# gargatik/Seamless-Through-Breaking-Rethinking-Image-Stitching-for-Optimal-Alignment

Measured on AMD Instinct MI355X. Metric: stitched image-pairs/s at 512x512, higher is better.
Workload: dtype f32 (decoder contractions, PatchEmbed's third conv and the C = 128 block tails: exact 3xbf16 split of both operands, 6 products on the bf16 matrix cores, fp32 accumulate -- error vs fp64 0.83x the fp32 MFMA chain's; everything else fp32); 1 GPU; UDIS-D-shaped 512x512 pairs, batch=1, FlowHomoAdpater.forward(type=test_eval); launch=hipGraph replay, pairs_in_flight=3

## Files before the change

### include/stitch_gfx950.h

```cpp
#ifndef STITCH_GFX950_H
#define STITCH_GFX950_H
#include <stdint.h>
#ifdef __cplusplus
extern "C" {
#endif

typedef struct st_gemm_desc {
    const float* a;
    const float* w;
    float* c;
    const float* bias;
    const float* aux0;
    const float* aux1;
    const float* aux2;
    const float* scale_ptr;
    int32_t M, N, K;
    int32_t H, W, Cin, ldx;
    int32_t kh, kw, sh, sw, ph, pw, Ho, Wo;
    int32_t ldw, ldc, ld_aux0, ld_aux1, ld_aux2;
    int32_t aux0_row_div, aux0_row_mod;
    int32_t act;
    int32_t epi;
    float alpha;
    int32_t batch;
// ... 124 lines not shown
int st_copy2d(const float* src, int32_t lds, float* dst, int32_t ldd, int32_t rows, int32_t cols, void* stream);
int st_prep_image(const float* src, float* dst, int32_t B, int32_t C, int32_t H, int32_t W, int32_t ldo,
                  float mul, float div, float sub, void* stream);

int st_latent_pool(const float* scores, int32_t ld_s, const float* tokens, int32_t ld_t, float* z, int32_t pixels,
                   int32_t P, void* stream);

int st_coords_grid(float* out, int32_t B, int32_t H, int32_t W, void* stream);
int st_coords_grid_init(float* out, const float* init, int32_t B, int32_t H, int32_t W, void* stream);
int st_flow_forward_interpolate(const float* src, int32_t src_is_coords_rows, float* out, int32_t B, int32_t H, int32_t W,
                                void* stream);
int st_flow_from_coords(const float* coords1, float* flow4, int32_t ld4, float* dst2, int32_t ld2, int32_t B,
                        int32_t H, int32_t W, void* stream);
int st_flow_encode(const float* coords1, const float* w98, const float* bias, float* out, int32_t ldo, float* flow2,
                   int32_t ld2, int32_t B, int32_t H, int32_t W, int32_t Co, void* stream);
int st_flow_encode_split3(const float* coords1, const float* w98, const float* bias, float* out, int32_t ldo, float* flow2,
                          int32_t ld2, int32_t B, int32_t H, int32_t W, int32_t Co, void* out_planes, int64_t out_pstride,
                          int64_t out_prows, void* flow_planes, int64_t flow_pstride, int64_t flow_prows, int32_t flow_col,
                          void* stream);
int st_cost_lookup(const float* maps, const float* coords, float* out, int32_t ldo, int32_t Nq, int32_t H2,
                   int32_t W2, int32_t r, void* stream);
int st_decoder_token_chain(float* corr, int32_t ld_corr, const float* coords1, const float* kv,
                           const float* const* weights16, int32_t rows, int32_t ntok, void* stream);
int st_convex_upsample(const float* coords1, const float* mask, int32_t ldm, float* out, int32_t B, int32_t H,
                       int32_t W, void* stream);

int st_dlt4(const float* src4x2, const float* motion, float* H, int32_t B, float mscale_x, float mscale_y,
            float div, void* stream);
int st_mat3_sandwich(const float* L, const float* X, const float* R, float* out, int32_t B, int32_t invert,
                     void* stream);
int st_homo_warp(const float* U, const float* theta, float* out, int32_t* idx, int32_t B, int32_t C,
                 int32_t n_ones, int32_t H, int32_t W, int32_t oh, int32_t ow, void* stream);
int st_mesh_bounds(const float* H, float* out4, int32_t B, float width, float height, int32_t gw, int32_t gh,
                   void* stream);
int st_flow_warp(const float* x, const float* flow, const float* mul, float* out, int32_t B, int32_t C,
                 int32_t H, int32_t W, void* stream);
int st_homo_flow_warp(const float* image2, const float* H8, const float* flow, float* out6, float* overlap, float* Hi,
                      int32_t B, int32_t H, int32_t W, void* stream);
int st_resize_bilinear(const float* x, float* out, int32_t planes, int32_t H, int32_t W, int32_t oh, int32_t ow,
                       int32_t align_corners, float div0, float div1, int32_t ndiv, void* stream);
int st_range_map(const float* flow, void* scratch_u64, float* out, int32_t B, int32_t H, int32_t W, void* stream);
int st_occlusion_from_range(const float* range, float* out, int64_t n, int32_t threshold, void* stream);
int st_morph_open(const float* mask, float* out, void* scratch_u8x2, int32_t N, int32_t H, int32_t W,
                  int32_t ksz, void* stream);
int st_eval_finish(float* final6, const float* occ, float* overlap, int32_t B, int32_t H, int32_t W, void* stream);
int st_blend(const float* homo1, const float* homo2, float* fin, const float* occ, float* output2, float* mask1,
// ... 169 lines not shown
```

### seamless-through-breaking-rethinking-image-stitching-for-optimal-alignment_amd/csrc/flowops.hip

```cpp
#include "common.h"
#include <type_traits>
#include "../../include/stitch_gfx950.h"

__global__ void coords_grid_kernel(float* __restrict__ out, int B, int H, int W) {
    const size_t idx = (size_t)blockIdx.x * blockDim.x + threadIdx.x;
    if (idx >= (size_t)B * H * W) return;
    const int r = idx % ((size_t)H * W);
    out[idx * 2] = (float)(r % W);
    out[idx * 2 + 1] = (float)(r / W);
}

extern "C" int st_coords_grid(float* out, int32_t B, int32_t H, int32_t W, void* stream) {
    if (!out || B <= 0 || H <= 0 || W <= 0) return ST_EINVAL;
    const size_t total = (size_t)B * H * W;
    hipLaunchKernelGGL(coords_grid_kernel, dim3((total + 255) / 256), dim3(256), 0, (hipStream_t)stream, out, B, H, W);
    ST_CHECK_LAUNCH();
    return ST_OK;
}

__global__ void coords_grid_init_kernel(float* __restrict__ out, const float* __restrict__ init, int B, int H, int W) {
    const size_t idx = (size_t)blockIdx.x * blockDim.x + threadIdx.x;
    if (idx >= (size_t)B * H * W) return;
    const size_t N = (size_t)H * W, b = idx / N;
    const int r = idx % N;
// ... 13 lines not shown
                                        float* __restrict__ dst2, int ld2, int B, int H, int W) {
    const size_t idx = (size_t)blockIdx.x * blockDim.x + threadIdx.x;
    if (idx >= (size_t)B * H * W) return;
    const int r = idx % ((size_t)H * W);
    const float fx = coords1[idx * 2] - (float)(r % W);
    const float fy = coords1[idx * 2 + 1] - (float)(r / W);
    if (flow4) {
        flow4[idx * ld4] = fx; flow4[idx * ld4 + 1] = fy;
        for (int c = 2; c < ld4; ++c) flow4[idx * ld4 + c] = 0.f;
    }
    if (dst2) { dst2[idx * ld2] = fx; dst2[idx * ld2 + 1] = fy; }
}

extern "C" int st_flow_from_coords(const float* coords1, float* flow4, int32_t ld4, float* dst2, int32_t ld2, int32_t B,
                                   int32_t H, int32_t W, void* stream) {
    if (!coords1 || B <= 0 || H <= 0 || W <= 0 || (flow4 && ld4 < 2) || (dst2 && ld2 < 2)) return ST_EINVAL;
    const size_t total = (size_t)B * H * W;
    hipLaunchKernelGGL(flow_from_coords_kernel, dim3((total + 255) / 256), dim3(256), 0, (hipStream_t)stream, coords1, flow4,
                       ld4, dst2, ld2, B, H, W);
    ST_CHECK_LAUNCH();
    return ST_OK;
}

__global__ __launch_bounds__(512) void flow_encode_kernel(const float* __restrict__ coords1, const float* __restrict__ w,
                                                          const float* __restrict__ bias, float* __restrict__ out, int ldo,
                                                          float* __restrict__ flow2, int ld2, int H, int W, int Co,
                                                          __bf16* __restrict__ out_planes, long long out_pstride, long long out_prows,
                                                          __bf16* __restrict__ flow_planes, long long flow_pstride, long long flow_prows, int flow_col) {
    __shared__ float2 patch[10 * 14];
    __shared__ __attribute__((aligned(16))) float wsm[98 * 128];
    const int tid = threadIdx.x, lane = tid & 63, wave = __builtin_amdgcn_readfirstlane(tid >> 6);
    const int tiles_x = (W + 7) >> 3;
    const int b = blockIdx.z, ty = (int)blockIdx.x / tiles_x, tx = (int)blockIdx.x - ty * tiles_x;
    const size_t img = (size_t)b * H * W;
    const int cbase = (int)blockIdx.y * 128;
    {
        float4 v[7];
#pragma unroll
        for (int u = 0; u < 7; ++u) {
            const int f = u * 512 + tid, t = f >> 5, c4 = (f & 31) * 4;
            v[u] = make_float4(0.f, 0.f, 0.f, 0.f);
            if (t < 98 && cbase + c4 < Co) v[u] = *reinterpret_cast<const float4*>(w + (size_t)t * Co + cbase + c4);
        }
#pragma unroll
        for (int u = 0; u < 7; ++u) {
            const int f = u * 512 + tid;
            if (f < 98 * 32) *reinterpret_cast<float4*>(wsm + f * 4) = v[u];
        }
    }
    if (tid < 140) {
        const int py = tid / 14, px = tid - py * 14;
        const int y = ty * 4 + py - 3, x = tx * 8 + px - 3;
        float2 f = make_float2(0.f, 0.f);
        if (y >= 0 && y < H && x >= 0 && x < W) {
            const float2 cc = *reinterpret_cast<const float2*>(coords1 + (img + (size_t)y * W + x) * 2);
            f = make_float2(cc.x - (float)x, cc.y - (float)y);
        }
        patch[tid] = f;
// ... 25 lines not shown
                acc[p] = fmaf(f[p + kx].y, wr[kx * 2 + 1], acc[p]);
            }
    }
#pragma unroll
    for (int p = 0; p < 8; ++p) {
        const int x = tx * 8 + p;
        if (x < W && cok) {
            const float o = fmaxf(acc[p], 0.f);
            out[(img + (size_t)y * W + x) * ldo + c] = o;
            if (out_planes) {
                __bf16 h, m, l;
                st_split3(o, h, m, l);
                const unsigned ph = st_bf16_bits(h), pm = st_bf16_bits(m), pl = st_bf16_bits(l);
                const unsigned nh = (unsigned)__builtin_amdgcn_update_dpp(0, (int)ph, 0xB1, 0xF, 0xF, false);
                const unsigned nm = (unsigned)__builtin_amdgcn_update_dpp(0, (int)pm, 0xB1, 0xF, 0xF, false);
                const unsigned nl = (unsigned)__builtin_amdgcn_update_dpp(0, (int)pl, 0xB1, 0xF, 0xF, false);
                if (!(c & 1)) {
                    unsigned* pp = reinterpret_cast<unsigned*>(out_planes + ((size_t)(c >> 5) * out_prows + img + (size_t)y * W + x) * 32 + (c & 31));
                    pp[0] = ph | (nh << 16); pp[out_pstride / 2] = pm | (nm << 16); pp[out_pstride] = pl | (nl << 16);
                }
            }
        }
    }
    if (flow2 && blockIdx.y == 0 && (wave & 1) == 0 && lane < 8 && tx * 8 + lane < W) {
        const float2 f = patch[(row + 3) * 14 + lane + 3];
        const size_t r = img + (size_t)y * W + tx * 8 + lane;
        flow2[r * ld2] = f.x; flow2[r * ld2 + 1] = f.y;
        if (flow_planes) {
            __bf16 hx, mx, lx, hy, my, ly;
            unsigned* pp = reinterpret_cast<unsigned*>(flow_planes + ((size_t)(flow_col >> 5) * flow_prows + r) * 32 + (flow_col & 31));
            st_split3(f.x, hx, mx, lx);
            st_split3(f.y, hy, my, ly);
            pp[0] = st_bf16_bits(hx) | ((unsigned)st_bf16_bits(hy) << 16);
            pp[flow_pstride / 2] = st_bf16_bits(mx) | ((unsigned)st_bf16_bits(my) << 16);
            pp[flow_pstride] = st_bf16_bits(lx) | ((unsigned)st_bf16_bits(ly) << 16);
        }
    }
}

extern "C" int st_flow_encode(const float* coords1, const float* w98, const float* bias, float* out, int32_t ldo, float* flow2,
                              int32_t ld2, int32_t B, int32_t H, int32_t W, int32_t Co, void* stream) {
    if (!coords1 || !w98 || !bias || !out || B <= 0 || H <= 0 || W <= 0 || Co <= 0 || (Co & 3) || ((uintptr_t)w98 & 15)) return ST_EINVAL;
    if (ldo < Co || (flow2 && ld2 < 2) || ((uintptr_t)coords1 & 7)) return ST_EINVAL;
    dim3 grid(((H + 3) / 4) * ((W + 7) / 8), (Co + 127) / 128, B);
    hipLaunchKernelGGL(flow_encode_kernel, grid, dim3(512), 0, (hipStream_t)stream, coords1, w98, bias, out, ldo, flow2, ld2, H, W, Co,
                       (__bf16*)nullptr, 0LL, 0LL, (__bf16*)nullptr, 0LL, 0LL, 0);
    ST_CHECK_LAUNCH();
    return ST_OK;
}

extern "C" int st_flow_encode_split3(const float* coords1, const float* w98, const float* bias, float* out, int32_t ldo, float* flow2,
                                     int32_t ld2, int32_t B, int32_t H, int32_t W, int32_t Co, void* out_planes, int64_t out_pstride,
                                     int64_t out_prows, void* flow_planes, int64_t flow_pstride, int64_t flow_prows, int32_t flow_col,
                                     void* stream) {
    if (!coords1 || !w98 || !bias || !out || B <= 0 || H <= 0 || W <= 0 || Co <= 0 || (Co & 31) || ((uintptr_t)w98 & 15)) return ST_EINVAL;
    if (ldo < Co || (flow2 && ld2 < 2) || ((uintptr_t)coords1 & 7)) return ST_EINVAL;
    if (!out_planes || out_pstride <= 0 || out_prows < (int64_t)B * H * W) return ST_EINVAL;
    if (flow_planes && (!flow2 || flow_pstride <= 0 || flow_prows < (int64_t)B * H * W || flow_col < 0 || (flow_col & 1))) return ST_EINVAL;
    dim3 grid(((H + 3) / 4) * ((W + 7) / 8), (Co + 127) / 128, B);
    hipLaunchKernelGGL(flow_encode_kernel, grid, dim3(512), 0, (hipStream_t)stream, coords1, w98, bias, out, ldo, flow2, ld2, H, W, Co,
                       (__bf16*)out_planes, (long long)out_pstride, (long long)out_prows, (__bf16*)flow_planes, (long long)flow_pstride,
                       (long long)flow_prows, (int)flow_col);
    ST_CHECK_LAUNCH();
    return ST_OK;
}

__global__ __launch_bounds__(256) void cost_lookup_kernel(const float* __restrict__ maps, const float* __restrict__ coords,
                                                          float* __restrict__ out, int ldo, int Nq, int H2, int W2, int r) {
#pragma clang fp contract(off)
    const int side = 2 * r + 1, nch = side * side;
    const size_t idx = (size_t)blockIdx.x * 256 + threadIdx.x;
    if (idx >= (size_t)Nq * nch) return;
    const int ch = idx % nch;
    const size_t n = idx / nch;
    const int i = ch / side, j = ch % side;
    const float x = coords[n * 2] + (float)(i - r);
    const float y = coords[n * 2 + 1] + (float)(j - r);
    const float gx = 2.0f * x / (float)(W2 - 1) - 1.0f, gy = 2.0f * y / (float)(H2 - 1) - 1.0f;
    const float ix = ((gx + 1.0f) / 2.0f) * (float)(W2 - 1), iy = ((gy + 1.0f) / 2.0f) * (float)(H2 - 1);
    const float x0f = floorf(ix), y0f = floorf(iy);
    const int x0 = (int)x0f, y0 = (int)y0f, x1 = x0 + 1, y1 = y0 + 1;
    const float x1f = x0f + 1.0f, y1f = y0f + 1.0f;
    const float nw = (x1f - ix) * (y1f - iy), ne = (ix - x0f) * (y1f - iy);
    const float sw = (x1f - ix) * (iy - y0f), se = (ix - x0f) * (iy - y0f);
    const float* m = maps + n * (size_t)(H2 * W2);
    const bool xin0 = x0 >= 0 && x0 < W2, xin1 = x1 >= 0 && x1 < W2;
    const bool yin0 = y0 >= 0 && y0 < H2, yin1 = y1 >= 0 && y1 < H2;
    float v = (xin0 && yin0 ? m[y0 * W2 + x0] : 0.f) * nw;
    v = __fmaf_rn(xin1 && yin0 ? m[y0 * W2 + x1] : 0.f, ne, v);
    v = __fmaf_rn(xin0 && yin1 ? m[y1 * W2 + x0] : 0.f, sw, v);
    v = __fmaf_rn(xin1 && yin1 ? m[y1 * W2 + x1] : 0.f, se, v);
    out[n * ldo + ch] = v;
}

extern "C" int st_cost_lookup(const float* maps, const float* coords, float* out, int32_t ldo, int32_t Nq, int32_t H2,
                              int32_t W2, int32_t r, void* stream) {
    if (!maps || !coords || !out || Nq <= 0 || r < 0 || r > 64 || ldo < (2 * r + 1) * (2 * r + 1)) return ST_EINVAL;
    if (H2 < 2 || W2 < 2 || (int64_t)H2 * W2 > 0x7fffffff) return ST_EINVAL;
    const size_t total = (size_t)Nq * (2 * r + 1) * (2 * r + 1);
    hipLaunchKernelGGL(cost_lookup_kernel, dim3((total + 255) / 256), dim3(256), 0, (hipStream_t)stream, maps, coords, out,
                       ldo, Nq, H2, W2, r);
    ST_CHECK_LAUNCH();
    return ST_OK;
}

__global__ __launch_bounds__(256) void convex_upsample_kernel(const float* __restrict__ coords1, const float* __restrict__ mask,
                                                              int ldm, float* __restrict__ out, int B, int H, int W) {
    const size_t gid = (size_t)blockIdx.x * 256 + threadIdx.x;
    const size_t pix = gid >> 6;
    if (pix >= (size_t)B * H * W) return;
    const int sub = gid & 63, i = sub >> 3, j = sub & 7;
    const int b = pix / ((size_t)H * W), r = pix % ((size_t)H * W);
    const int y = r / W, x = r % W;
    const float* mp = mask + pix * ldm + sub;
    float mv[9], mx = -INFINITY;
// ... 82 lines not shown
    for (int r = 0; r < 4; ++r) {
        mh[r] = sum16(v[0][r] + v[1][r]) * (1.0f / 32.0f);
        const float d0 = v[0][r] - mh[r], d1 = v[1][r] - mh[r];
        m2h[r] = sum16(d0 * d0 + d1 * d1);
        if (c == 0) { red_mine[(4 * g + r) * 2] = mh[r]; red_mine[(4 * g + r) * 2 + 1] = m2h[r]; }
    }
    __syncthreads();
#pragma unroll
    for (int r = 0; r < 4; ++r) {
        const float mo = red_other[(4 * g + r) * 2], m2o = red_other[(4 * g + r) * 2 + 1];
        const float mean = 0.5f * (mh[r] + mo), d = mh[r] - mo;
        const float var = ((m2h[r] + m2o) + d * d * 16.0f) * (1.0f / 64.0f);
        const float rstd = 1.0f / sqrtf(var + 1e-5f);
#pragma unroll
        for (int t = 0; t < 2; ++t) v[t][r] = (v[t][r] - mean) * rstd * w[col0 + 16 * t + c] + b[col0 + 16 * t + c];
    }
}

template <int I, int N, class F>
__device__ __forceinline__ void tc_static_for(F&& f) {
    if constexpr (I < N) { f(std::integral_constant<int, I>{}); tc_static_for<I + 1, N>(f); }
}

template <int RG>
__global__ __launch_bounds__(128 * RG) void decoder_token_chain_kernel(float* __restrict__ corr, int ldc, const float* __restrict__ coords1,
                                                                       const float* __restrict__ kv, TokenChainArgs A, int rows, int ntok) {
    extern __shared__ __attribute__((aligned(16))) float sm[];
    float* W0 = sm;
    float* W2 = W0 + 64 * TC_LDW0;
    float* Wq = W2 + 64 * TC_LDW;
    float* Wp = Wq + 64 * TC_LDW;
    float* Wf0 = Wp + 64 * TC_LDW;
    float* Wf3 = Wf0 + 64 * TC_LDW;
    float* Vec = Wf3 + 64 * TC_LDW;
    float* Slab = Vec + 10 * 64;
    float* Red = Slab + RG * 16 * (TC_LDW0 + TC_LDW);
    const int tid = threadIdx.x, lane = tid & 63, wave = tid >> 6;
    constexpr int NT = 128 * RG;
    const int rg = wave >> 1, hf = wave & 1, col0 = 32 * hf;
    float* S0 = Slab + rg * 16 * (TC_LDW0 + TC_LDW);
    float* S1 = S0 + 16 * TC_LDW0;
    float* red_mine = Red + (rg * 2 + hf) * 32;
    const float* red_other = Red + (rg * 2 + (hf ^ 1)) * 32;
    const int row0 = (blockIdx.x * RG + rg) * 16;
    const int c = lane & 15, g = lane >> 4;
    const int jmax = ntok - 1;

    constexpr int P0 = 1536 / NT, P1 = 1024 / NT;
    float4 xv[3], w0v[P0];
    f32x4 wv[5 * P1], vecv;
    float cx[4], cy[4];
    {
        const int e = min(tid, 159), q = e >> 4;
        const float* vp = q == 0 ? A.b0 : q == 1 ? A.b2 : q == 2 ? A.n1w : q == 3 ? A.n1b : q == 4 ? A.bq : q == 5 ? A.bp : q == 6 ? A.n2w
                          : q == 7 ? A.n2b : q == 8 ? A.bf0 : A.bf3;
        vecv = *reinterpret_cast<const f32x4*>(vp + 4 * (e & 15));
    }
    tc_static_for<0, 3>([&](auto ic) {
        constexpr int i = decltype(ic)::value;
        const int e = (hf * 64 + lane) + 128 * i, r = e / 24, k4 = e % 24;
        xv[i] = *reinterpret_cast<const float4*>(corr + (size_t)min(row0 + r, rows - 1) * ldc + 4 * min(k4, 20));
    });
    tc_static_for<0, P0>([&](auto ic) {
        constexpr int i = decltype(ic)::value;
        const int e = tid + NT * i, n = e / 24, k4 = e % 24;
        w0v[i] = *reinterpret_cast<const float4*>(A.w0 + n * 84 + 4 * min(k4, 20));
    });
    tc_static_for<0, P1>([&](auto ic) {
        constexpr int i = decltype(ic)::value;
        const int off = 4 * (tid + NT * i);
        wv[5 * i + 0] = *reinterpret_cast<const f32x4*>(A.w2 + off);
        wv[5 * i + 1] = *reinterpret_cast<const f32x4*>(A.wq + off);
        wv[5 * i + 2] = *reinterpret_cast<const f32x4*>(A.wp + off);
        wv[5 * i + 3] = *reinterpret_cast<const f32x4*>(A.wf0 + off);
        wv[5 * i + 4] = *reinterpret_cast<const f32x4*>(A.wf3 + off);
    });
#pragma unroll
    for (int r = 0; r < 4; ++r) {
        const float2 p2 = *reinterpret_cast<const float2*>(coords1 + (size_t)min(row0 + 4 * g + r, rows - 1) * 2);
        cx[r] = p2.x; cy[r] = p2.y;
    }
    tc_static_for<0, 3>([&](auto ic) {
        constexpr int i = decltype(ic)::value;
        const int e = (hf * 64 + lane) + 128 * i, r = e / 24, k4 = e % 24;
        *reinterpret_cast<float4*>(S0 + r * TC_LDW0 + 4 * k4) = k4 < 21 ? xv[i] : make_float4(0.f, 0.f, 0.f, 0.f);
    });
    tc_static_for<0, P0>([&](auto ic) {
        constexpr int i = decltype(ic)::value;
        const int e = tid + NT * i, n = e / 24, k4 = e % 24;
        *reinterpret_cast<float4*>(W0 + n * TC_LDW0 + 4 * k4) = k4 < 21 ? w0v[i] : make_float4(0.f, 0.f, 0.f, 0.f);
    });
    tc_static_for<0, P1>([&](auto ic) {
        constexpr int i = decltype(ic)::value;
        const int e = tid + NT * i, n = e >> 4, k4 = e & 15, off = n * TC_LDW + 4 * k4;
        *reinterpret_cast<f32x4*>(W2 + off) = wv[5 * i + 0];
        *reinterpret_cast<f32x4*>(Wq + off) = wv[5 * i + 1];
        *reinterpret_cast<f32x4*>(Wp + off) = wv[5 * i + 2];
        *reinterpret_cast<f32x4*>(Wf0 + off) = wv[5 * i + 3];
        *reinterpret_cast<f32x4*>(Wf3 + off) = wv[5 * i + 4];
    });
    if (tid < 160) *reinterpret_cast<f32x4*>(Vec + 4 * tid) = vecv;
    asm volatile("" ::: "memory");
    const int head = 4 * hf + g;
    float4 kk[8][2], vv[8][2];
    {
        const float* kvr = kv + (size_t)min(row0 + c, rows - 1) * ntok * 128 + 8 * head;
#pragma unroll
        for (int j = 0; j < 8; ++j)
#pragma unroll
            for (int e = 0; e < 2; ++e) kk[j][e] = *reinterpret_cast<const float4*>(kvr + min(j, jmax) * 128 + 4 * e);
#pragma unroll
        for (int j = 0; j < 8; ++j)
#pragma unroll
            for (int e = 0; e < 2; ++e) vv[j][e] = *reinterpret_cast<const float4*>(kvr + min(j, jmax) * 128 + 64 + 4 * e);
    }
    asm volatile("" ::: "memory");
    __syncthreads();
    const float *b0 = Vec, *b2 = Vec + 64, *n1w = Vec + 128, *n1b = Vec + 192, *bq = Vec + 256, *bp = Vec + 320, *n2w = Vec + 384,
                *n2b = Vec + 448, *bf0 = Vec + 512, *bf3 = Vec + 576;
    f32x4 acc[2], query[2], x[2];
    tc_gemm2<96, TC_LDW0, TC_LDW0>(S0, W0 + col0 * TC_LDW0, acc, lane);
#pragma unroll
    for (int t = 0; t < 2; ++t)
#pragma unroll
        for (int r = 0; r < 4; ++r) acc[t][r] = st_act(acc[t][r] + b0[col0 + 16 * t + c], ST_ACT_GELU);
    tc_store2(S1, acc, col0, lane);
    __syncthreads();
    tc_gemm2<64, TC_LDW, TC_LDW>(S1, W2 + col0 * TC_LDW, query, lane);
#pragma unroll
    for (int t = 0; t < 2; ++t)
#pragma unroll
        for (int r = 0; r < 4; ++r) query[t][r] += b2[col0 + 16 * t + c];
#pragma unroll
    for (int t = 0; t < 2; ++t) acc[t] = query[t];
    tc_layernorm2(acc, n1w, n1b, red_mine, red_other, col0, lane);
#pragma unroll
    for (int r = 0; r < 4; ++r) {
        const float a = ((3.14f * (hf ? cy[r] : cx[r])) * (float)c) * 0.005f;
        acc[0][r] += sinf(a); acc[1][r] += cosf(a);
// ... 51 lines not shown
        for (int r = 0; r < 4; ++r) x[t][r] = query[t][r] + (acc[t][r] + bp[col0 + 16 * t + c]);
#pragma unroll
    for (int t = 0; t < 2; ++t) acc[t] = x[t];
    tc_layernorm2(acc, n2w, n2b, red_mine, red_other, col0, lane);
    tc_store2(S0, acc, col0, lane);
    __syncthreads();
    tc_gemm2<64, TC_LDW, TC_LDW>(S0, Wf0 + col0 * TC_LDW, acc, lane);
#pragma unroll
    for (int t = 0; t < 2; ++t)
#pragma unroll
        for (int r = 0; r < 4; ++r) acc[t][r] = st_act(acc[t][r] + bf0[col0 + 16 * t + c], ST_ACT_GELU);
    tc_store2(S1, acc, col0, lane);
    __syncthreads();
    tc_gemm2<64, TC_LDW, TC_LDW>(S1, Wf3 + col0 * TC_LDW, acc, lane);
#pragma unroll
    for (int t = 0; t < 2; ++t)
#pragma unroll
        for (int r = 0; r < 4; ++r) {
            const int row = row0 + 4 * g + r;
            if (row < rows) corr[(size_t)row * ldc + 84 + col0 + 16 * t + c] = x[t][r] + (acc[t][r] + bf3[col0 + 16 * t + c]);
        }
}

extern "C" int st_decoder_token_chain(float* corr, int32_t ld_corr, const float* coords1, const float* kv, const float* const* weights16,
                                      int32_t rows, int32_t ntok, void* stream) {
    if (!corr || !coords1 || !kv || !weights16 || rows <= 0 || ntok <= 0 || ntok > 8 || ld_corr < 148 || (ld_corr & 3)) return ST_EINVAL;
    TokenChainArgs A;
    const float** dst = reinterpret_cast<const float**>(&A);
    for (int i = 0; i < 16; ++i) { if (!weights16[i]) return ST_EINVAL; dst[i] = weights16[i]; }
    constexpr int RG = 4;
    const size_t lds = (size_t)(64 * TC_LDW0 + 5 * 64 * TC_LDW + 640 + RG * 16 * (TC_LDW0 + TC_LDW) + RG * 64) * sizeof(float);
    (void)hipFuncSetAttribute((const void*)decoder_token_chain_kernel<RG>, hipFuncAttributeMaxDynamicSharedMemorySize, (int)lds);
    hipLaunchKernelGGL(decoder_token_chain_kernel<RG>, dim3((rows + 16 * RG - 1) / (16 * RG)), dim3(128 * RG), lds, (hipStream_t)stream, corr, ld_corr,
                       coords1, kv, A, rows, ntok);
    ST_CHECK_LAUNCH();
    return ST_OK;
}
```

### seamless-through-breaking-rethinking-image-stitching-for-optimal-alignment_amd/flowformer.py

```python
from __future__ import annotations

import os

import torch
import torch.nn as nn

from . import ops
from .checkpoint import HP, ParamTree, flat_params, flow_spec
from .homography import pack_conv


SPLIT3 = os.environ.get("ST_SPLIT3", "1") != "0"


def _new(rows, cols, dev, zero=False):
    return (torch.zeros if zero else torch.empty)((rows, cols), device=dev, dtype=torch.float32)


def _planes_copy(p):
    return ops.Planes(p.rows, p.C, None, t=p.t.clone(), c0=p.c0, ncols=p.ncols)


def _keep(trace, **named):
    if trace is None:
# ... 443 lines not shown
            x = self._vertical(pk["vert"][i], x, ctx, B, H1, W1, nl, extra_res=short if i == HP["encoder_depth"] - 1 else None)
            _keep(trace, vert=[x])
        return x

    def _gru_tables(self, inp, B, H1, W1):
        D = self._pk["dec"]
        gru_geom = {"1": (B, H1, W1, 1, 5, 1, 1, 0, 2), "2": (B, H1, W1, 5, 1, 1, 1, 2, 0)}
        tabs = {}
        for sfx in ("1", "2"):
            tabs[sfx] = _new(inp.shape[0], 384, inp.device)
            ops.conv_gemm(inp, D["inp" + sfx][0], tabs[sfx], geom=gru_geom[sfx], bias=D["inp" + sfx][1])
        return tabs

    def _update_state(self, R, B, N, dev):
        S = dict(hxA=_new(R, 384, dev), hxB=_new(R, 384, dev), corr=_new(R, 160, dev, zero=True),
                 cor1=_new(R, 256, dev), corflo=_new(R, 256, dev), flo1=_new(R, 128, dev),
                 vT=torch.empty((B, 128, N), device=dev), zbuf=_new(R, 128, dev), fh=_new(R, 256, dev))
        S["s3"] = SPLIT3 and N % 32 == 0 and "s3" in self._pk["dec"]
        if S["s3"]:
            S.update(hxA_p=ops.Planes(R, 384, dev), hxB_p=ops.Planes(R, 384, dev), cor1_p=ops.Planes(R, 256, dev), flo1_p=ops.Planes(R, 128, dev),
                     corflo_p=ops.Planes(R, 256, dev))
        return S

    def _update_block(self, S, coords1, attn, gru_tab, B, H1, W1, trace=None):
        D = self._pk["dec"]
        N = H1 * W1
        s3 = S["s3"]
        hxA = S["hxA"]
        net, motion, flow, agg = hxA[:, :128], hxA[:, 128:254], hxA[:, 254:256], hxA[:, 256:]
        g3 = (B, H1, W1, 3, 3, 1, 1, 1, 1)
        _keep(trace, coords_in=coords1, net_in=net)
        ops.conv_gemm(S["corr"], D["convc1"][0], S["cor1"], bias=D["convc1"][1], act="relu", **_emit(S, "cor1", 0, 256))
        enc = (coords1, D["convf1"][0], D["convf1"][1], S["flo1"], flow, B, H1, W1)
        if s3:
            ops.flow_encode_split3(*enc, S["flo1_p"], (S["hxA_p"], 254))
        else:
            ops.flow_encode(*enc)
        ops.conv_gemm_pair((_act(S, "cor1", 0, 256), _wt(D, S, "convc2"), S["corflo"][:, :192],
                            dict(geom=g3, bias=D["convc2"][1], act="relu", **_emit(S, "corflo", 0, 192, no_f32=True))),
                           (_act(S, "flo1", 0, 128), _wt(D, S, "convf2"), S["corflo"][:, 192:],
                            dict(geom=g3, bias=D["convf2"][1], act="relu", **_emit(S, "corflo", 192, 256, no_f32=True))))
        corflo = _act(S, "corflo", 0, 256)
        _keep(trace, cor1=S["cor1"], flo1=S["flo1"], flow=flow, **{"corflo_p" if s3 else "corflo": corflo})
        ops.conv_gemm(corflo, _wt(D, S, "conv"), motion, geom=g3, bias=D["conv"][1], act="relu", **_emit(S, "hxA", 128, 256))
        _keep(trace, motion=motion)
        ops.gma_aggregate(attn, hxA[:, 128:256], D["to_v"], D["gamma"], S["vT"], agg, B, N, **_emit(S, "hxA", 256, 384))
        _keep(trace, aggregate=agg)
        gru = (S["zbuf"], gru_tab["1"], gru_tab["2"], *((D["s3"] if s3 else D)[k] for k in ("zr1", "q1", "zr2", "q2")), B, H1, W1)
        if s3:
            ops.sepconv_gru_split3(hxA, S["hxA_p"], S["hxB_p"], *gru)
        else:
            ops.sepconv_gru(hxA, S["hxB"], *gru)
        _keep(trace, gru=net)
        ops.conv_gemm(_act(S, "hxA", 0, 128), _wt(D, S, "fh1"), S["fh"], geom=g3, bias=D["fh1"][1], act="relu")
        ops.conv_gemm(S["fh"], D["fh2"][0], coords1, geom=g3, bias=D["fh2"][1], epi="add", aux1=coords1)
        _keep(trace, fh=S["fh"], coords_out=coords1, hxA=hxA)
        if s3:
# ... 20 lines not shown
        qk = _new(R, 256, dev)
        attn = torch.empty((B, N, N), device=dev)
        ops.gma_attention(inp, D["qk"], qk, attn, B, N)
        _keep(trace, net=S["hxA"][:, :128], inp=inp, gru_tab=gru_tab, attn=attn, qk=qk)
        if S["s3"]:
            _keep(trace, net_p=S["hxA_p"])
        return dict(S=S, inp=inp, gru_tab=gru_tab, attn=attn, qk=qk)

    def _decoder(self, mem, ctx, cost_maps, B, H1, W1, iters, trace=None, flow_init=None):
        D = self._pk["dec"]
        dev = ctx.device
        N = H1 * W1
        R = B * N
        nl = self._pk["latents"].shape[0]
        pro = None if trace is None else trace[-1].setdefault("prologue", {})
        pre = self._decoder_prologue(ctx, B, H1, W1, trace=pro)
        S, gru_tab, attn = pre["S"], pre["gru_tab"], pre["attn"]
        kv = _new(R * nl, 128, dev)
        ops.conv_gemm(mem, D["ca"]["kv"][0], kv, bias=D["ca"]["kv"][1])
        _keep(pro, kv=kv)
        coords1 = _new(R, 2, dev)
        ops.coords_grid(coords1, B, H1, W1, init=flow_init)
        for it in range(iters):
            ops.cost_lookup9x9(cost_maps, coords1, S["corr"], R, H1, W1)
            ops.decoder_token_chain(S["corr"], coords1, kv, D["chain16"], R, nl)
            rec = _record(trace)
            self._update_block(S, coords1, attn, gru_tab, B, H1, W1, trace=rec)
            _keep(rec, coords1=coords1, net=S["hxA"][:, :128], corr=S["corr"])
        last = None if trace is None else trace[-1]
        mask = self._mask_head(S, B, H1, W1, trace=last)
        flow_up = torch.empty((B, 2, 8 * H1, 8 * W1), device=dev)
        ops.convex_upsample(coords1, mask, flow_up, B, H1, W1)
        _keep(last, mask=mask, flow_up=flow_up)
        return flow_up, coords1

    def _forward(self, image1, image2, iters, trace, flow_init, pair):
        if not image1.is_cuda:
            raise RuntimeError("FlowFormer runs on the MI355X HIP kernels only: move the module and inputs to cuda")
        pk = self._pk or self.pack()
        iters = HP["decoder_depth"] if iters is None else iters
        B, _, H, W = image1.shape
        if H % 32 or W % 32:
            raise RuntimeError(f"input size {H}x{W} must be a multiple of 32 (reference runs both nets at 512x512)")
        dev = image1.device
        Bd = 2 * B if pair else B
        tr = None if trace is None else dict(cnet=[], fnet=[], encoder={})
        x = _new(2 * B * H * W, 4, dev)
        ops.prep_image(image1.contiguous(), x[:B * H * W], 4, 2.0, 255.0, 1.0)
        ops.prep_image(image2.contiguous(), x[B * H * W:], 4, 2.0, 255.0, 1.0)
        ctx, H1, W1 = self._twins(pk["cnet"], x if pair else x[:B * H * W], Bd, H, W, trace=tr and tr["cnet"])
# ... 37 lines not shown
```

### seamless-through-breaking-rethinking-image-stitching-for-optimal-alignment_amd/ops.py

```python
from __future__ import annotations

import ctypes as C

import torch

from ._lib import ChainDesc, GemmDesc, JpegDecParams, JpegEncParams, MlpDesc, check, lib
from .jpeg_probe import JpegInfo, probe as _jpeg_probe
from ._lib import StitchError as StitchErrorBase

ACT = dict(none=0, relu=1, gelu=2, sigmoid=3, tanh=4, lrelu=5)
EPI = dict(store=0, add=1, mul=2, gru=3, axpy=4, zr=5)

assert lib.st_abi_gemm_desc_size() == C.sizeof(GemmDesc), "st_gemm_desc ABI mismatch between header and binding"
assert lib.st_abi_chain_desc_size() == C.sizeof(ChainDesc), "st_chain_desc ABI mismatch between header and binding"
assert lib.st_abi_mlp_desc_size() == C.sizeof(MlpDesc), "st_mlp_desc ABI mismatch between header and binding"
assert lib.st_abi_jpeg_dec_params_size() == C.sizeof(JpegDecParams), "st_jpeg_dec_params ABI mismatch between header and binding"
assert lib.st_abi_jpeg_enc_params_size() == C.sizeof(JpegEncParams), "st_jpeg_enc_params ABI mismatch between header and binding"


def _stream():
    return C.c_void_p(torch.cuda.current_stream().cuda_stream)


def _p(t):
# ... 415 lines not shown
                             B, H, W, w98.shape[1], _stream()), "st_flow_encode")
    return out


def flow_encode_split3(coords1, w98, bias, out, flow2, B, H, W, out_planes, flow_planes):
    fp, fcol = flow_planes
    check(lib.st_flow_encode_split3(_pc(coords1), _pc(w98), _pc(bias), _p(out), _ld(out), _p(flow2), _ld(flow2), B, H, W, w98.shape[1],
                                    C.c_void_p(out_planes.ptr()), out_planes.pstride, out_planes.rows,
                                    C.c_void_p(fp.t.data_ptr()), fp.pstride, fp.rows, int(fcol), _stream()), "st_flow_encode_split3")
    return out


def cost_lookup(maps, coords, out, Nq, H2, W2, r=4):
    check(lib.st_cost_lookup(_p(maps), _p(coords), _p(out), _ld(out), Nq, H2, W2, r, _stream()), "st_cost_lookup")
    return out


def decoder_token_chain(corr, coords1, kv, weights16, rows, ntok):
    arr = (C.c_void_p * 16)(*[w.data_ptr() for w in weights16])
    check(lib.st_decoder_token_chain(_p(corr), _ld(corr), _pc(coords1), _p(kv), arr, rows, ntok, _stream()), "st_decoder_token_chain")
    return corr


def _ws(dev):
    ws = _workspace(dev)
    return ws.data_ptr(), ws.numel()


def patch_conv12(maps, c0_w, c0_b, c2_w, c2_b, out, M, H=64, W=64):
    check(lib.st_patch_conv12(_pc(maps), _pc(c0_w), _pc(c0_b), _pc(c2_w), _pc(c2_b), _p(out), M, H, W, _stream()), "st_patch_conv12")
    return out


def patch_conv12_planes(maps, c0_w, c0_b, c2_w, c2_b, planes, M, H=64, W=64):
    check(lib.st_patch_conv12_planes(_pc(maps), _pc(c0_w), _pc(c0_b), _pc(c2_w), _pc(c2_b), C.c_void_p(planes.ptr()), planes.pstride, M, H, W, _stream()),
          "st_patch_conv12_planes")
    return planes


def cost_lookup9x9(maps, coords, out, Nq, H2, W2):
    check(lib.st_cost_lookup9x9(_p(maps), _pc(coords), _p(out), _ld(out), Nq, H2, W2, _stream()), "st_cost_lookup9x9")
    return out


def patch_embed(cost_maps, weights11, ld_f0, pe_bias, s1, s2, s3, s4, tokens, M, H, W):
    arr = (C.c_void_p * 11)(*[w.data_ptr() for w in weights11])
# ... 855 lines not shown
```

Baseline: 98.42 pairs/s.

## Fuse cost lookup, decoder token chain and flow encode into one decoder-head kernel

Adds a decoder_head kernel whose blocks either run the token chain with the 9x9 cost lookup computed in-kernel (gathering bilinear samples straight into LDS) or run the flow-encode conv, selected by block index. This replaces three launches per decoder iteration with one and removes the corr round-trip through global memory before the chain reads it. In exchange, the flow-encode blocks now run with the chain's larger LDS allocation and launch bounds, which can lower their occupancy. Heterogeneous blocks in one grid may also balance unevenly.

```diff
diff --git a/include/stitch_gfx950.h b/include/stitch_gfx950.h
--- a/include/stitch_gfx950.h
+++ b/include/stitch_gfx950.h
@@ -170,6 +170,11 @@
                    int32_t W2, int32_t r, void* stream);
 int st_decoder_token_chain(float* corr, int32_t ld_corr, const float* coords1, const float* kv,
                            const float* const* weights16, int32_t rows, int32_t ntok, void* stream);
+int st_decoder_head(const float* cost_maps, int32_t H2, int32_t W2, float* corr, int32_t ld_corr, const float* coords1,
+                    const float* kv, const float* const* weights16, int32_t rows, int32_t ntok, const float* w98, const float* bias,
+                    float* flo, int32_t ld_flo, float* flow2, int32_t ld2, int32_t B, int32_t H, int32_t W, int32_t Co,
+                    void* flo_planes, int64_t flo_pstride, int64_t flo_prows, void* flow_planes, int64_t flow_pstride,
+                    int64_t flow_prows, int32_t flow_col, void* stream);
 int st_convex_upsample(const float* coords1, const float* mask, int32_t ldm, float* out, int32_t B, int32_t H,
                        int32_t W, void* stream);
 
diff --git a/seamless-through-breaking-rethinking-image-stitching-for-optimal-alignment_amd/csrc/flowops.hip b/seamless-through-breaking-rethinking-image-stitching-for-optimal-alignment_amd/csrc/flowops.hip
--- a/seamless-through-breaking-rethinking-image-stitching-for-optimal-alignment_amd/csrc/flowops.hip
+++ b/seamless-through-breaking-rethinking-image-stitching-for-optimal-alignment_amd/csrc/flowops.hip
@@ -59,18 +59,30 @@
     return ST_OK;
 }
 
-__global__ __launch_bounds__(512) void flow_encode_kernel(const float* __restrict__ coords1, const float* __restrict__ w,
-                                                          const float* __restrict__ bias, float* __restrict__ out, int ldo,
-                                                          float* __restrict__ flow2, int ld2, int H, int W, int Co,
-                                                          __bf16* __restrict__ out_planes, long long out_pstride, long long out_prows,
-                                                          __bf16* __restrict__ flow_planes, long long flow_pstride, long long flow_prows, int flow_col) {
-    __shared__ float2 patch[10 * 14];
-    __shared__ __attribute__((aligned(16))) float wsm[98 * 128];
+struct FlowEncodeArgs {
+    const float *coords1, *w, *bias;
+    float* out;
+    int ldo;
+    float* flow2;
+    int ld2, H, W, Co;
+    __bf16* out_planes;
+    long long out_pstride, out_prows;
+    __bf16* flow_planes;
+    long long flow_pstride, flow_prows;
+    int flow_col;
+};
+
+__device__ __forceinline__ void flow_encode_body(float2* __restrict__ patch, float* __restrict__ wsm, int tile, int cblk, int b,
+                                                 const float* __restrict__ coords1, const float* __restrict__ w,
+                                                 const float* __restrict__ bias, float* __restrict__ out, int ldo,
+                                                 float* __restrict__ flow2, int ld2, int H, int W, int Co,
+                                                 __bf16* __restrict__ out_planes, long long out_pstride, long long out_prows,
+                                                 __bf16* __restrict__ flow_planes, long long flow_pstride, long long flow_prows, int flow_col) {
     const int tid = threadIdx.x, lane = tid & 63, wave = __builtin_amdgcn_readfirstlane(tid >> 6);
     const int tiles_x = (W + 7) >> 3;
-    const int b = blockIdx.z, ty = (int)blockIdx.x / tiles_x, tx = (int)blockIdx.x - ty * tiles_x;
+    const int ty = tile / tiles_x, tx = tile - ty * tiles_x;
     const size_t img = (size_t)b * H * W;
-    const int cbase = (int)blockIdx.y * 128;
+    const int cbase = cblk * 128;
     {
         float4 v[7];
 #pragma unroll
@@ -142,7 +154,7 @@
             }
         }
     }
-    if (flow2 && blockIdx.y == 0 && (wave & 1) == 0 && lane < 8 && tx * 8 + lane < W) {
+    if (flow2 && cblk == 0 && (wave & 1) == 0 && lane < 8 && tx * 8 + lane < W) {
         const float2 f = patch[(row + 3) * 14 + lane + 3];
         const size_t r = img + (size_t)y * W + tx * 8 + lane;
         flow2[r * ld2] = f.x; flow2[r * ld2 + 1] = f.y;
@@ -156,6 +168,17 @@
             pp[flow_pstride] = st_bf16_bits(lx) | ((unsigned)st_bf16_bits(ly) << 16);
         }
     }
+}
+
+__global__ __launch_bounds__(512) void flow_encode_kernel(const float* __restrict__ coords1, const float* __restrict__ w,
+                                                          const float* __restrict__ bias, float* __restrict__ out, int ldo,
+                                                          float* __restrict__ flow2, int ld2, int H, int W, int Co,
+                                                          __bf16* __restrict__ out_planes, long long out_pstride, long long out_prows,
+                                                          __bf16* __restrict__ flow_planes, long long flow_pstride, long long flow_prows, int flow_col) {
+    __shared__ float2 patch[10 * 14];
+    __shared__ __attribute__((aligned(16))) float wsm[98 * 128];
+    flow_encode_body(patch, wsm, (int)blockIdx.x, (int)blockIdx.y, (int)blockIdx.z, coords1, w, bias, out, ldo, flow2, ld2, H, W, Co, out_planes,
+                     out_pstride, out_prows, flow_planes, flow_pstride, flow_prows, flow_col);
 }
 
 extern "C" int st_flow_encode(const float* coords1, const float* w98, const float* bias, float* out, int32_t ldo, float* flow2,
@@ -185,32 +208,47 @@
     return ST_OK;
 }
 
+struct LookupAxis {
+    float w0, w1;
+    int p0;
+};
+
+__device__ __forceinline__ LookupAxis lookup_axis(float c, int off, int size) {
+#pragma clang fp contract(off)
+    const float x = c + (float)off;
+    const float g = 2.0f * x / (float)(size - 1) - 1.0f;
+    const float ix = ((g + 1.0f) / 2.0f) * (float)(size - 1);
+    const float f0 = floorf(ix), f1 = f0 + 1.0f;
+    LookupAxis a;
+    a.w0 = f1 - ix; a.w1 = ix - f0; a.p0 = (int)f0;
+    return a;
+}
+
+__device__ __forceinline__ float lookup_blend(const LookupAxis& ax, const LookupAxis& ay, float vnw, float vne, float vsw, float vse) {
+#pragma clang fp contract(off)
+    const float nw = ax.w0 * ay.w0, ne = ax.w1 * ay.w0, sw = ax.w0 * ay.w1, se = ax.w1 * ay.w1;
+    float v = vnw * nw;
+    v = __fmaf_rn(vne, ne, v);
+    v = __fmaf_rn(vsw, sw, v);
+    v = __fmaf_rn(vse, se, v);
+    return v;
+}
+
 __global__ __launch_bounds__(256) void cost_lookup_kernel(const float* __restrict__ maps, const float* __restrict__ coords,
                                                           float* __restrict__ out, int ldo, int Nq, int H2, int W2, int r) {
-#pragma clang fp contract(off)
     const int side = 2 * r + 1, nch = side * side;
     const size_t idx = (size_t)blockIdx.x * 256 + threadIdx.x;
     if (idx >= (size_t)Nq * nch) return;
     const int ch = idx % nch;
     const size_t n = idx / nch;
     const int i = ch / side, j = ch % side;
-    const float x = coords[n * 2] + (float)(i - r);
-    const float y = coords[n * 2 + 1] + (float)(j - r);
-    const float gx = 2.0f * x / (float)(W2 - 1) - 1.0f, gy = 2.0f * y / (float)(H2 - 1) - 1.0f;
-    const float ix = ((gx + 1.0f) / 2.0f) * (float)(W2 - 1), iy = ((gy + 1.0f) / 2.0f) * (float)(H2 - 1);
-    const float x0f = floorf(ix), y0f = floorf(iy);
-    const int x0 = (int)x0f, y0 = (int)y0f, x1 = x0 + 1, y1 = y0 + 1;
-    const float x1f = x0f + 1.0f, y1f = y0f + 1.0f;
-    const float nw = (x1f - ix) * (y1f - iy), ne = (ix - x0f) * (y1f - iy);
-    const float sw = (x1f - ix) * (iy - y0f), se = (ix - x0f) * (iy - y0f);
+    const LookupAxis ax = lookup_axis(coords[n * 2], i - r, W2), ay = lookup_axis(coords[n * 2 + 1], j - r, H2);
+    const int x0 = ax.p0, y0 = ay.p0, x1 = x0 + 1, y1 = y0 + 1;
     const float* m = maps + n * (size_t)(H2 * W2);
     const bool xin0 = x0 >= 0 && x0 < W2, xin1 = x1 >= 0 && x1 < W2;
     const bool yin0 = y0 >= 0 && y0 < H2, yin1 = y1 >= 0 && y1 < H2;
-    float v = (xin0 && yin0 ? m[y0 * W2 + x0] : 0.f) * nw;
-    v = __fmaf_rn(xin1 && yin0 ? m[y0 * W2 + x1] : 0.f, ne, v);
-    v = __fmaf_rn(xin0 && yin1 ? m[y1 * W2 + x0] : 0.f, sw, v);
-    v = __fmaf_rn(xin1 && yin1 ? m[y1 * W2 + x1] : 0.f, se, v);
-    out[n * ldo + ch] = v;
+    out[n * ldo + ch] = lookup_blend(ax, ay, xin0 && yin0 ? m[y0 * W2 + x0] : 0.f, xin1 && yin0 ? m[y0 * W2 + x1] : 0.f,
+                                     xin0 && yin1 ? m[y1 * W2 + x0] : 0.f, xin1 && yin1 ? m[y1 * W2 + x1] : 0.f);
 }
 
 extern "C" int st_cost_lookup(const float* maps, const float* coords, float* out, int32_t ldo, int32_t Nq, int32_t H2,
@@ -339,10 +377,10 @@
     if constexpr (I < N) { f(std::integral_constant<int, I>{}); tc_static_for<I + 1, N>(f); }
 }
 
-template <int RG>
-__global__ __launch_bounds__(128 * RG) void decoder_token_chain_kernel(float* __restrict__ corr, int ldc, const float* __restrict__ coords1,
-                                                                       const float* __restrict__ kv, TokenChainArgs A, int rows, int ntok) {
-    extern __shared__ __attribute__((aligned(16))) float sm[];
+template <int RG, bool LOOKUP>
+__device__ __forceinline__ void token_chain_body(float* __restrict__ sm, int blk, float* __restrict__ corr, int ldc, const float* __restrict__ coords1,
+                                                 const float* __restrict__ kv, TokenChainArgs A, int rows, int ntok,
+                                                 const float* __restrict__ maps, int mH, int mW) {
     float* W0 = sm;
     float* W2 = W0 + 64 * TC_LDW0;
     float* Wq = W2 + 64 * TC_LDW;
@@ -359,9 +397,18 @@
     float* S1 = S0 + 16 * TC_LDW0;
     float* red_mine = Red + (rg * 2 + hf) * 32;
     const float* red_other = Red + (rg * 2 + (hf ^ 1)) * 32;
-    const int row0 = (blockIdx.x * RG + rg) * 16;
+    const int row0 = (blk * RG + rg) * 16;
     const int c = lane & 15, g = lane >> 4;
     const int jmax = ntok - 1;
+
+    constexpr int NS = 11;
+    const int lrow = tid >> 3, ls = tid & 7;
+    const int lgrow = blk * 16 * RG + lrow, ln = min(lgrow, rows - 1);
+    float2 lc = make_float2(0.f, 0.f);
+    if constexpr (LOOKUP) {
+        static_assert(NT == 8 * 16 * RG, "eight threads per row");
+        lc = *reinterpret_cast<const float2*>(coords1 + (size_t)ln * 2);
+    }
 
     constexpr int P0 = 1536 / NT, P1 = 1024 / NT;
     float4 xv[3], w0v[P0];
@@ -373,11 +420,12 @@
                           : q == 7 ? A.n2b : q == 8 ? A.bf0 : A.bf3;
         vecv = *reinterpret_cast<const f32x4*>(vp + 4 * (e & 15));
     }
-    tc_static_for<0, 3>([&](auto ic) {
-        constexpr int i = decltype(ic)::value;
-        const int e = (hf * 64 + lane) + 128 * i, r = e / 24, k4 = e % 24;
-        xv[i] = *reinterpret_cast<const float4*>(corr + (size_t)min(row0 + r, rows - 1) * ldc + 4 * min(k4, 20));
-    });
+    if constexpr (!LOOKUP)
+        tc_static_for<0, 3>([&](auto ic) {
+            constexpr int i = decltype(ic)::value;
+            const int e = (hf * 64 + lane) + 128 * i, r = e / 24, k4 = e % 24;
+            xv[i] = *reinterpret_cast<const float4*>(corr + (size_t)min(row0 + r, rows - 1) * ldc + 4 * min(k4, 20));
+        });
     tc_static_for<0, P0>([&](auto ic) {
         constexpr int i = decltype(ic)::value;
         const int e = tid + NT * i, n = e / 24, k4 = e % 24;
@@ -397,11 +445,34 @@
         const float2 p2 = *reinterpret_cast<const float2*>(coords1 + (size_t)min(row0 + 4 * g + r, rows - 1) * 2);
         cx[r] = p2.x; cy[r] = p2.y;
     }
-    tc_static_for<0, 3>([&](auto ic) {
-        constexpr int i = decltype(ic)::value;
-        const int e = (hf * 64 + lane) + 128 * i, r = e / 24, k4 = e % 24;
-        *reinterpret_cast<float4*>(S0 + r * TC_LDW0 + 4 * k4) = k4 < 21 ? xv[i] : make_float4(0.f, 0.f, 0.f, 0.f);
-    });
+    float* ltab = Slab + (lrow >> 4) * 16 * (TC_LDW0 + TC_LDW) + 16 * TC_LDW0 + (lrow & 15) * TC_LDW;
+    float lg[NS][4];
+    if constexpr (LOOKUP) {
+        asm volatile("" ::: "memory");
+#pragma unroll
+        for (int u = 0; u < 3; ++u) {
+            const int e = min(ls + 8 * u, 17);
+            const LookupAxis a = e < 9 ? lookup_axis(lc.x, e - 4, mW) : lookup_axis(lc.y, e - 13, mH);
+            if (ls + 8 * u < 18) { ltab[3 * e] = a.w0; ltab[3 * e + 1] = a.w1; ltab[3 * e + 2] = __int_as_float(a.p0); }
+        }
+        __builtin_amdgcn_wave_barrier();
+        const float* m = maps + (size_t)ln * (size_t)(mH * mW);
+        tc_static_for<0, NS>([&](auto kc) {
+            constexpr int k = decltype(kc)::value;
+            const int q = min(ls + 8 * k, 80), j = q / 9, i = q - 9 * j;
+            const int x0 = __float_as_int(ltab[3 * i + 2]), y0 = __float_as_int(ltab[3 * (9 + j) + 2]), x1 = x0 + 1, y1 = y0 + 1;
+            const int xa = x0 >= 0 && x0 < mW ? x0 : 0, xb = x1 >= 0 && x1 < mW ? x1 : 0;
+            const int ya = y0 >= 0 && y0 < mH ? y0 : 0, yb = y1 >= 0 && y1 < mH ? y1 : 0;
+            lg[k][0] = m[ya * mW + xa]; lg[k][1] = m[ya * mW + xb]; lg[k][2] = m[yb * mW + xa]; lg[k][3] = m[yb * mW + xb];
+        });
+        asm volatile("" ::: "memory");
+    }
+    if constexpr (!LOOKUP)
+        tc_static_for<0, 3>([&](auto ic) {
+            constexpr int i = decltype(ic)::value;
+            const int e = (hf * 64 + lane) + 128 * i, r = e / 24, k4 = e % 24;
+            *reinterpret_cast<float4*>(S0 + r * TC_LDW0 + 4 * k4) = k4 < 21 ? xv[i] : make_float4(0.f, 0.f, 0.f, 0.f);
+        });
     tc_static_for<0, P0>([&](auto ic) {
         constexpr int i = decltype(ic)::value;
         const int e = tid + NT * i, n = e / 24, k4 = e % 24;
@@ -432,6 +503,24 @@
             for (int e = 0; e < 2; ++e) vv[j][e] = *reinterpret_cast<const float4*>(kvr + min(j, jmax) * 128 + 64 + 4 * e);
     }
     asm volatile("" ::: "memory");
+    if constexpr (LOOKUP) {
+        float* s0row = Slab + (lrow >> 4) * 16 * (TC_LDW0 + TC_LDW) + (lrow & 15) * TC_LDW0;
+        tc_static_for<0, NS>([&](auto kc) {
+            constexpr int k = decltype(kc)::value;
+            const int qr = ls + 8 * k, q = min(qr, 80), j = q / 9, i = q - 9 * j, ch = 9 * i + j;
+            LookupAxis ax, ay;
+            ax.w0 = ltab[3 * i]; ax.w1 = ltab[3 * i + 1]; ax.p0 = __float_as_int(ltab[3 * i + 2]);
+            ay.w0 = ltab[3 * (9 + j)]; ay.w1 = ltab[3 * (9 + j) + 1]; ay.p0 = __float_as_int(ltab[3 * (9 + j) + 2]);
+            const int x0 = ax.p0, y0 = ay.p0, x1 = x0 + 1, y1 = y0 + 1;
+            const bool xin0 = x0 >= 0 && x0 < mW, xin1 = x1 >= 0 && x1 < mW;
+            const bool yin0 = y0 >= 0 && y0 < mH, yin1 = y1 >= 0 && y1 < mH;
+            const float v = lookup_blend(ax, ay, xin0 && yin0 ? lg[k][0] : 0.f, xin1 && yin0 ? lg[k][1] : 0.f,
+                                         xin0 && yin1 ? lg[k][2] : 0.f, xin1 && yin1 ? lg[k][3] : 0.f);
+            if (qr < 81 && lgrow < rows) corr[(size_t)lgrow * ldc + ch] = v;
+            s0row[qr < 81 ? ch : qr] = qr < 81 ? v : 0.f;
+        });
+        s0row[88 + ls] = 0.f;
+    }
     __syncthreads();
     const float *b0 = Vec, *b2 = Vec + 64, *n1w = Vec + 128, *n1b = Vec + 192, *bq = Vec + 256, *bp = Vec + 320, *n2w = Vec + 384,
                 *n2b = Vec + 448, *bf0 = Vec + 512, *bf3 = Vec + 576;
@@ -529,6 +618,18 @@
         }
 }
 
+template <int RG>
+__global__ __launch_bounds__(128 * RG) void decoder_token_chain_kernel(float* __restrict__ corr, int ldc, const float* __restrict__ coords1,
+                                                                       const float* __restrict__ kv, TokenChainArgs A, int rows, int ntok) {
+    extern __shared__ __attribute__((aligned(16))) float sm[];
+    token_chain_body<RG, false>(sm, (int)blockIdx.x, corr, ldc, coords1, kv, A, rows, ntok, nullptr, 0, 0);
+}
+
+template <int RG>
+static size_t token_chain_lds_bytes() {
+    return (size_t)(64 * TC_LDW0 + 5 * 64 * TC_LDW + 640 + RG * 16 * (TC_LDW0 + TC_LDW) + RG * 64) * sizeof(float);
+}
+
 extern "C" int st_decoder_token_chain(float* corr, int32_t ld_corr, const float* coords1, const float* kv, const float* const* weights16,
                                       int32_t rows, int32_t ntok, void* stream) {
     if (!corr || !coords1 || !kv || !weights16 || rows <= 0 || ntok <= 0 || ntok > 8 || ld_corr < 148 || (ld_corr & 3)) return ST_EINVAL;
@@ -536,10 +637,56 @@
     const float** dst = reinterpret_cast<const float**>(&A);
     for (int i = 0; i < 16; ++i) { if (!weights16[i]) return ST_EINVAL; dst[i] = weights16[i]; }
     constexpr int RG = 4;
-    const size_t lds = (size_t)(64 * TC_LDW0 + 5 * 64 * TC_LDW + 640 + RG * 16 * (TC_LDW0 + TC_LDW) + RG * 64) * sizeof(float);
+    const size_t lds = token_chain_lds_bytes<RG>();
     (void)hipFuncSetAttribute((const void*)decoder_token_chain_kernel<RG>, hipFuncAttributeMaxDynamicSharedMemorySize, (int)lds);
     hipLaunchKernelGGL(decoder_token_chain_kernel<RG>, dim3((rows + 16 * RG - 1) / (16 * RG)), dim3(128 * RG), lds, (hipStream_t)stream, corr, ld_corr,
                        coords1, kv, A, rows, ntok);
     ST_CHECK_LAUNCH();
     return ST_OK;
 }
+
+template <int RG>
+__global__ __launch_bounds__(128 * RG) void decoder_head_kernel(const float* __restrict__ maps, int H2, int W2, float* __restrict__ corr, int ldc,
+                                                                const float* __restrict__ coords1, const float* __restrict__ kv, TokenChainArgs A,
+                                                                int rows, int ntok, FlowEncodeArgs F, int n_chain, int flow_tiles, int flow_cblks) {
+    extern __shared__ __attribute__((aligned(16))) float sm[];
+    const int blk = (int)blockIdx.x;
+    if (blk < n_chain) {
+        token_chain_body<RG, true>(sm, blk, corr, ldc, coords1, kv, A, rows, ntok, maps, H2, W2);
+    } else {
+        const int u = blk - n_chain, per_b = flow_tiles * flow_cblks, b = u / per_b, v = u - b * per_b, cblk = v / flow_tiles;
+        flow_encode_body(reinterpret_cast<float2*>(sm), sm + 2 * 10 * 14, v - cblk * flow_tiles, cblk, b, F.coords1, F.w, F.bias, F.out, F.ldo,
+                         F.flow2, F.ld2, F.H, F.W, F.Co, F.out_planes, F.out_pstride, F.out_prows, F.flow_planes, F.flow_pstride, F.flow_prows,
+                         F.flow_col);
+    }
+}
+
+extern "C" int st_decoder_head(const float* cost_maps, int32_t H2, int32_t W2, float* corr, int32_t ld_corr, const float* coords1,
+                               const float* kv, const float* const* weights16, int32_t rows, int32_t ntok, const float* w98, const float* bias,
+                               float* flo, int32_t ld_flo, float* flow2, int32_t ld2, int32_t B, int32_t H, int32_t W, int32_t Co,
+                               void* flo_planes, int64_t flo_pstride, int64_t flo_prows, void* flow_planes, int64_t flow_pstride,
+                               int64_t flow_prows, int32_t flow_col, void* stream) {
+    if (!cost_maps || H2 < 2 || W2 < 2 || (int64_t)H2 * W2 > 0x7fffffff) return ST_EINVAL;
+    if (!corr || !coords1 || !kv || !weights16 || rows <= 0 || ntok <= 0 || ntok > 8 || ld_corr < 148 || (ld_corr & 3)) return ST_EINVAL;
+    if (!w98 || !bias || !flo || B <= 0 || H <= 0 || W <= 0 || Co <= 0 || (Co & (flo_planes ? 31 : 3)) || ((uintptr_t)w98 & 15)) return ST_EINVAL;
+    if (ld_flo < Co || (flow2 && ld2 < 2) || ((uintptr_t)coords1 & 7)) return ST_EINVAL;
+    if ((int64_t)B * H * W != rows) return ST_EINVAL;
+    if (flo_planes ? (flo_pstride <= 0 || flo_prows < rows) : flow_planes != nullptr) return ST_EINVAL;
+    if (flow_planes && (!flow2 || flow_pstride <= 0 || flow_prows < rows || flow_col < 0 || (flow_col & 1))) return ST_EINVAL;
+    TokenChainArgs A;
+    const float** dst = reinterpret_cast<const float**>(&A);
+    for (int i = 0; i < 16; ++i) { if (!weights16[i]) return ST_EINVAL; dst[i] = weights16[i]; }
+    constexpr int RG = 4;
+    const int n_chain = (rows + 16 * RG - 1) / (16 * RG), flow_tiles = ((H + 3) / 4) * ((W + 7) / 8), flow_cblks = (Co + 127) / 128;
+    const int64_t n_flow = (int64_t)flow_tiles * flow_cblks * B;
+    if (n_chain + n_flow > 0x7fffffff) return ST_EINVAL;
+    const FlowEncodeArgs F = {coords1, w98, bias, flo, ld_flo, flow2, ld2, H, W, Co, (__bf16*)flo_planes, (long long)flo_pstride, (long long)flo_prows,
+                              (__bf16*)flow_planes, (long long)flow_pstride, (long long)flow_prows, (int)flow_col};
+    const size_t lds = token_chain_lds_bytes<RG>();
+    static_assert((2 * 10 * 14 + 98 * 128) * sizeof(float) <= (64 * TC_LDW0 + 5 * 64 * TC_LDW) * sizeof(float), "the flow encode's LDS fits the chain's block");
+    (void)hipFuncSetAttribute((const void*)decoder_head_kernel<RG>, hipFuncAttributeMaxDynamicSharedMemorySize, (int)lds);
+    hipLaunchKernelGGL(decoder_head_kernel<RG>, dim3((unsigned)(n_chain + n_flow)), dim3(128 * RG), lds, (hipStream_t)stream, cost_maps, (int)H2, (int)W2,
+                       corr, ld_corr, coords1, kv, A, rows, ntok, F, n_chain, flow_tiles, flow_cblks);
+    ST_CHECK_LAUNCH();
+    return ST_OK;
+}
diff --git a/seamless-through-breaking-rethinking-image-stitching-for-optimal-alignment_amd/flowformer.py b/seamless-through-breaking-rethinking-image-stitching-for-optimal-alignment_amd/flowformer.py
--- a/seamless-through-breaking-rethinking-image-stitching-for-optimal-alignment_amd/flowformer.py
+++ b/seamless-through-breaking-rethinking-image-stitching-for-optimal-alignment_amd/flowformer.py
@@ -489,7 +489,7 @@
                      corflo_p=ops.Planes(R, 256, dev))
         return S
 
-    def _update_block(self, S, coords1, attn, gru_tab, B, H1, W1, trace=None):
+    def _update_block(self, S, coords1, attn, gru_tab, B, H1, W1, trace=None, encoded=False):
         D = self._pk["dec"]
         N = H1 * W1
         s3 = S["s3"]
@@ -499,7 +499,9 @@
         _keep(trace, coords_in=coords1, net_in=net)
         ops.conv_gemm(S["corr"], D["convc1"][0], S["cor1"], bias=D["convc1"][1], act="relu", **_emit(S, "cor1", 0, 256))
         enc = (coords1, D["convf1"][0], D["convf1"][1], S["flo1"], flow, B, H1, W1)
-        if s3:
+        if encoded:
+            pass
+        elif s3:
             ops.flow_encode_split3(*enc, S["flo1_p"], (S["hxA_p"], 254))
         else:
             ops.flow_encode(*enc)
@@ -566,10 +568,10 @@
         coords1 = _new(R, 2, dev)
         ops.coords_grid(coords1, B, H1, W1, init=flow_init)
         for it in range(iters):
-            ops.cost_lookup9x9(cost_maps, coords1, S["corr"], R, H1, W1)
-            ops.decoder_token_chain(S["corr"], coords1, kv, D["chain16"], R, nl)
+            ops.decoder_head(cost_maps, H1, W1, S["corr"], coords1, kv, D["chain16"], R, nl, D["convf1"][0], D["convf1"][1], S["flo1"],
+                             S["hxA"][:, 254:256], B, H1, W1, *((S["flo1_p"], (S["hxA_p"], 254)) if S["s3"] else ()))
             rec = _record(trace)
-            self._update_block(S, coords1, attn, gru_tab, B, H1, W1, trace=rec)
+            self._update_block(S, coords1, attn, gru_tab, B, H1, W1, trace=rec, encoded=True)
             _keep(rec, coords1=coords1, net=S["hxA"][:, :128], corr=S["corr"])
         last = None if trace is None else trace[-1]
         mask = self._mask_head(S, B, H1, W1, trace=last)
diff --git a/seamless-through-breaking-rethinking-image-stitching-for-optimal-alignment_amd/ops.py b/seamless-through-breaking-rethinking-image-stitching-for-optimal-alignment_amd/ops.py
--- a/seamless-through-breaking-rethinking-image-stitching-for-optimal-alignment_amd/ops.py
+++ b/seamless-through-breaking-rethinking-image-stitching-for-optimal-alignment_amd/ops.py
@@ -461,6 +461,27 @@
     return corr
 
 
+def decoder_head(cost_maps, H2, W2, corr, coords1, kv, weights16, rows, ntok, w98, bias, flo, flow2, B, H, W, flo_planes=None, flow_planes=None):
+    arr = (C.c_void_p * 16)(*[w.data_ptr() for w in weights16])
+    fp, fcol = flow_planes if flow_planes is not None else (None, 0)
+    rc = lib.st_decoder_head(_pc(cost_maps), H2, W2, _p(corr), _ld(corr), _pc(coords1), _p(kv), arr, rows, ntok, _pc(w98), _pc(bias),
+                             _p(flo), _ld(flo), _p(flow2), _ld(flow2) if flow2 is not None else 0, B, H, W, w98.shape[1],
+                             C.c_void_p(flo_planes.ptr()) if flo_planes is not None else None,
+                             flo_planes.pstride if flo_planes is not None else 0, flo_planes.rows if flo_planes is not None else 0,
+                             C.c_void_p(fp.t.data_ptr()) if fp is not None else None, fp.pstride if fp is not None else 0,
+                             fp.rows if fp is not None else 0, int(fcol), _stream())
+    if rc == 1001:
+        cost_lookup9x9(cost_maps, coords1, corr, rows, H2, W2)
+        decoder_token_chain(corr, coords1, kv, weights16, rows, ntok)
+        if flo_planes is not None:
+            flow_encode_split3(coords1, w98, bias, flo, flow2, B, H, W, flo_planes, flow_planes)
+        else:
+            flow_encode(coords1, w98, bias, flo, flow2, B, H, W)
+        return corr
+    check(rc, "st_decoder_head")
+    return corr
+
+
 def _ws(dev):
     ws = _workspace(dev)
     return ws.data_ptr(), ws.numel()
```

Result: no change. 98.55 pairs/s, median of 6 (+0.1%).
